# zeux/calm

Hardware: NVIDIA B200
Metric: tok/s single-batch decode (higher is better)
Workload: dtype f32 (fp8 e5m2 weights, f32 accumulate, fp16 KV)

## Files before the change

### calm_b200/csrc/attn.cuh

```cuda
#pragma once

#include "stages.cuh"

#define ATTN2_BP 16
#define ATTN2_MAXB 32

__device__ __forceinline__ void cluster_sync_all() {
	asm volatile("barrier.cluster.arrive.release.aligned;" ::: "memory");
	asm volatile("barrier.cluster.wait.acquire.aligned;" ::: "memory");
}
__device__ __forceinline__ float ld_dsmem(const float* local_ptr, uint32_t cta_rank) {
	uint32_t raddr;
	float v;
	asm volatile("mapa.shared::cluster.u32 %0, %1, %2;" : "=r"(raddr) : "r"(smem_u32(local_ptr)), "r"(cta_rank));
	asm volatile("ld.shared::cluster.f32 %0, [%1];" : "=f"(v) : "r"(raddr) : "memory");
	return v;
}

#define ATTN2_MAX_CLUSTER 16

template <typename KVT>
__host__ __device__ inline size_t attn2_smem_bytes(int hg, int head_dim, int nbmax, int nsplit) {
	size_t kv = (size_t)2 * nbmax * ATTN2_BP * head_dim * sizeof(KVT);
	size_t scratch = (size_t)(ATTN_THREADS / 32) * hg * (head_dim + 2);
	size_t scratch2 = (size_t)(2 * nsplit + 1) * hg;
	if (scratch2 > scratch) scratch = scratch2;
	return kv + ((size_t)hg * head_dim + scratch + (size_t)hg * (head_dim + 2)) * sizeof(float);
}

__device__ __forceinline__ float attn_cell_wait(const unsigned long long* cell, unsigned epoch, int* err) {
	unsigned long long v;
	unsigned spins = 0;
	unsigned long long t0 = 0;
	for (;;) {
		asm volatile("ld.volatile.global.u64 %0, [%1];" : "=l"(v) : "l"(cell) : "memory");
		if ((unsigned)(v >> 32) == epoch) break;
		if ((++spins & 1023) == 0) {
			const unsigned long long now = globaltimer_ns();
			if (!t0) t0 = now;
			if (now - t0 > 5000000000ull) {
				if (err) *reinterpret_cast<volatile int*>(err) = 9200;
				__threadfence_system();
				__trap();
			}
		}
	}
	return __uint_as_float((unsigned)v);
}

__device__ __forceinline__ void attn_cell_pair_wait(const unsigned long long* cell, unsigned epoch, int* err, float& v0, float& v1) {
	unsigned long long c0, c1;
	unsigned spins = 0;
	unsigned long long t0 = 0;
	for (;;) {
		asm volatile("ld.volatile.global.v2.u64 {%0, %1}, [%2];" : "=l"(c0), "=l"(c1) : "l"(cell) : "memory");
		if ((unsigned)(c0 >> 32) == epoch && (unsigned)(c1 >> 32) == epoch) break;
		if ((++spins & 1023) == 0) {
			const unsigned long long now = globaltimer_ns();
			if (!t0) t0 = now;
			if (now - t0 > 5000000000ull) {
				if (err) *reinterpret_cast<volatile int*>(err) = 9201;
				__threadfence_system();
				__trap();
			}
		}
	}
	v0 = __uint_as_float((unsigned)c0), v1 = __uint_as_float((unsigned)c1);
}

template <typename KVT, int HG, int LPP, bool CLUSTER>
__global__ void __launch_bounds__(ATTN_THREADS) k_attn2(const AttnArgs a) {
	typedef typename KvRaw<KVT>::type raw_t;
	constexpr int HD = LPP * 8, P = LPP / HG, G = 32 / LPP, NW = ATTN_THREADS / 32, NC = LPP;
	static_assert(HG * P == LPP && P >= 1 && P <= 4 && ATTN2_BP % P == 0, "unsupported head grouping");
	extern __shared__ __align__(128) unsigned char smem_raw[];
	__shared__ __align__(8) uint64_t bars[ATTN2_MAXB];
	__shared__ int flag;
	const int tid = threadIdx.x, lane = tid & 31, warp = tid >> 5;
	const int nbmax = a.nbmax, nsplit = a.nsplit;
	const int unit = blockIdx.x / nsplit, split = blockIdx.x % nsplit;
	const int kvh = unit / a.qgroups;
	const int hbase = kvh * a.kv_mul + (unit % a.qgroups) * HG;
	constexpr uint32_t BLK = ATTN2_BP * HD * sizeof(KVT);
	KVT* Ks = reinterpret_cast<KVT*>(smem_raw);
	KVT* Vs = Ks + (size_t)nbmax * ATTN2_BP * HD;
	float* qs = reinterpret_cast<float*>(Vs + (size_t)nbmax * ATTN2_BP * HD);
	float* scratch = qs + HG * HD;
	float* myrec = scratch + max(NW * HG * (HD + 2), (2 * nsplit + 1) * HG);
	const KVT* kglob = reinterpret_cast<const KVT*>(a.kc) + (size_t)kvh * a.seq_len * HD;
	const KVT* vglob = reinterpret_cast<const KVT*>(a.vc) + (size_t)kvh * a.seq_len * HD;

#define ATTN_DBG(i)                                                          \
	do {                                                                     \
		if (a.dbg && blockIdx.x == 0 && tid == 0) a.dbg[i] = globaltimer_ns(); \
	} while (0)
	ATTN_DBG(0);
	pdl_launch_next();
	if (tid == 0) {
		for (int j = 0; j < nbmax; ++j) mbar_init(&bars[j], 1);
		mbar_init_fence();
	}
	__syncthreads();
	bool issued = false;
	auto request = [&](int j) {
		const int b = split + j * nsplit;
		const uint32_t bytes = (uint32_t)min(ATTN2_BP, a.seq_len - b * ATTN2_BP) * HD * sizeof(KVT);
		mbar_expect_tx(&bars[j], 2 * bytes);
		tma_load_1d(Ks + (size_t)j * ATTN2_BP * HD, kglob + (size_t)b * ATTN2_BP * HD, bytes, &bars[j]);
		tma_load_1d(Vs + (size_t)j * ATTN2_BP * HD, vglob + (size_t)b * ATTN2_BP * HD, bytes, &bars[j]);
	};
	if (tid < nbmax) {
		const int hint = min(*reinterpret_cast<const volatile int*>(&a.tp->kv_len), a.seq_len);
		if ((split + tid * nsplit) * ATTN2_BP < hint) request(tid), issued = true;
	}
	pdl_wait_prev();
	stamp_begin(a.stamp);
	ATTN_DBG(1);
	if (a.dbg && tid == 0) atomicMin(a.dbg + 10, globaltimer_ns());
	constexpr int QPT = (HG * HD + ATTN_THREADS - 1) / ATTN_THREADS;
	float qreg[QPT];
#pragma unroll
	for (int i = 0; i < QPT; ++i) qreg[i] = (tid + i * ATTN_THREADS < HG * HD) ? __ldcg(a.q + (size_t)hbase * HD + tid + i * ATTN_THREADS) : 0.f;
	const int kv_len = a.tp->kv_len, kv_pos = a.tp->kv_pos, kv_sink = a.tp->kv_sink;
	const unsigned epoch = (unsigned)a.tp->tp_seq * a.epoch_stride + a.epoch_idx;
	if (tid < nbmax && !issued && (split + tid * nsplit) * ATTN2_BP < kv_len) request(tid), issued = true;
#pragma unroll
	for (int i = 0; i < QPT; ++i)
		if (tid + i * ATTN_THREADS < HG * HD) qs[tid + i * ATTN_THREADS] = qreg[i];
	__syncthreads();
	ATTN_DBG(2);

	const int nblk = (kv_len + ATTN2_BP - 1) / ATTN2_BP;
	const int nb = nblk > split ? (nblk - split + nsplit - 1) / nsplit : 0;
	const int nslots = nb * ATTN2_BP;
	const int grp = lane / LPP, li = lane % LPP;

	float acc[HG][8], m[HG], l[HG];
#pragma unroll
	for (int h = 0; h < HG; ++h) {
		m[h] = -FLT_MAX, l[h] = 0.f;
#pragma unroll
		for (int d = 0; d < 8; ++d) acc[h][d] = 0.f;
	}
	float mh = -FLT_MAX, lh = 0.f;

	constexpr int SC = 4, STEP = NW * G * P;
	const int gbase = grp * LPP;
	auto slot_of = [&](int s0, int& j, int& o, int& t0) {
// ... 106 lines not shown
				for (int e = 0; e < 8; ++e) {
					float v = acc[h][e];
#pragma unroll
					for (int i = 0; i < P; ++i) v = fmaf(pw[i], vf[i][e], v);
					acc[h][e] = v;
				}
			}
		}
	}
	ATTN_DBG(4);
#pragma unroll
	for (int h = 0; h < HG; ++h) {
		m[h] = __shfl_sync(0xffffffffu, mh, grp * LPP + h * P);
		l[h] = __shfl_sync(0xffffffffu, lh, grp * LPP + h * P);
	}
	if constexpr (CLUSTER) {
		constexpr int REC = HD + 2;
		__shared__ float mls[ATTN2_MAX_CLUSTER][HG][2];
		__shared__ float invl[HG];
		attn_cta_merge<HG>(a, HG, 0, HG, warp, NW, m, l, acc, scratch, myrec);
		cluster_sync_all();
		for (int i = tid; i < nsplit * HG; i += ATTN_THREADS) {
			const int s = i / HG, h = i % HG;
			mls[s][h][0] = ld_dsmem(myrec + h * REC + HD, s), mls[s][h][1] = ld_dsmem(myrec + h * REC + HD + 1, s);
		}
		__syncthreads();
		if (tid < HG) {
			float M = -FLT_MAX;
			for (int s = 0; s < nsplit; ++s) M = fmaxf(M, mls[s][tid][0]);
			float L = 0.f;
			for (int s = 0; s < nsplit; ++s) {
				const float c = expf(mls[s][tid][0] - M);
				L = fmaf(mls[s][tid][1], c, L);
				mls[s][tid][0] = c;
			}
			invl[tid] = 1.0f / L;
		}
		__syncthreads();
		const int nout = HG * HD, per = (nout + nsplit - 1) / nsplit;
		const int o_end = min(nout, (split + 1) * per);
		for (int o0 = split * per; o0 < o_end; o0 += ATTN_THREADS / 8) {
			const int o = o0 + tid / 8, sg = tid & 7;
			float v = 0.f;
			if (o < o_end) {
				const int h = o / HD, e = o % HD;
				for (int s = sg; s < nsplit; s += 8) v = fmaf(ld_dsmem(myrec + h * REC + e, s), mls[s][h][0], v);
			}
			v += __shfl_xor_sync(0xffffffffu, v, 1), v += __shfl_xor_sync(0xffffffffu, v, 2), v += __shfl_xor_sync(0xffffffffu, v, 4);
			if (o < o_end && sg == 0) __stcg(a.out + (size_t)hbase * HD + o, v * invl[o / HD]);
		}
		cluster_sync_all();
	} else {
		constexpr int REC = HD + 2;
		__shared__ float mls[ATTN2_MAXB + 4][HG][2];
		__shared__ float invl[HG];
		(void)flag;
		attn_cta_merge<HG>(a, HG, 0, HG, warp, NW, m, l, acc, scratch, myrec);
		__syncthreads();
		ATTN_DBG(5);
		unsigned long long* cells = a.cells + (size_t)unit * nsplit * HG * REC;
		for (int i = tid; i < HG * REC; i += ATTN_THREADS) {
			const unsigned long long c = ((unsigned long long)epoch << 32) | __float_as_uint(myrec[i]);
			asm volatile("st.volatile.global.u64 [%0], %1;" ::"l"(cells + (size_t)split * HG * REC + i), "l"(c) : "memory");
		}
		for (int i = tid; i < nsplit * HG; i += ATTN_THREADS) {
			const int s = i / HG, h = i % HG;
			const unsigned long long* c = cells + (size_t)s * HG * REC + h * REC + HD;
			if (s == split) mls[s][h][0] = myrec[h * REC + HD], mls[s][h][1] = myrec[h * REC + HD + 1];
			else attn_cell_pair_wait(c, epoch, a.err, mls[s][h][0], mls[s][h][1]);
		}
		__syncthreads();
		__shared__ float cfs[ATTN2_MAXB + 4][HG];
		for (int i = tid; i < nsplit * HG; i += ATTN_THREADS) {
			const int s = i / HG, h = i % HG;
			float M = -FLT_MAX;
			for (int s2 = 0; s2 < nsplit; ++s2) M = fmaxf(M, mls[s2][h][0]);
			cfs[s][h] = expf(mls[s][h][0] - M);
		}
		__syncthreads();
		if (tid < HG) {
			float L = 0.f;
			for (int s = 0; s < nsplit; ++s) L = fmaf(mls[s][tid][1], cfs[s][tid], L);
			invl[tid] = 1.0f / L;
		}
		for (int i = tid; i < nsplit * HG; i += ATTN_THREADS) mls[i / HG][i % HG][0] = cfs[i / HG][i % HG];
		__syncthreads();
		ATTN_DBG(6);
		const int nout = HG * HD, per = (nout + nsplit - 1) / nsplit;
		const int o_end = min(nout, (split + 1) * per);
		for (int o0 = split * per; o0 < o_end; o0 += ATTN_THREADS / 8) {
			const int o = o0 + tid / 8, sg = tid & 7;
			float v = 0.f;
			if (o < o_end) {
				const int h = o / HD, e = o % HD;
				constexpr int NS8 = (ATTN2_MAXB + 4 + 7) / 8;
				unsigned long long c[NS8];
#pragma unroll
				for (int k = 0; k < NS8; ++k) {
					const int s = sg + 8 * k;
					c[k] = 0;
					if (s < nsplit && s != split) asm volatile("ld.volatile.global.u64 %0, [%1];" : "=l"(c[k]) : "l"(cells + (size_t)s * HG * REC + h * REC + e) : "memory");
				}
#pragma unroll
				for (int k = 0; k < NS8; ++k) {
					const int s = sg + 8 * k;
					if (s < nsplit) {
						float x;
						if (s == split) x = myrec[h * REC + e];
						else if ((unsigned)(c[k] >> 32) == epoch) x = __uint_as_float((unsigned)c[k]);
						else x = attn_cell_wait(cells + (size_t)s * HG * REC + h * REC + e, epoch, a.err);
						v = fmaf(x, mls[s][h][0], v);
					}
				}
			}
			v += __shfl_xor_sync(0xffffffffu, v, 1), v += __shfl_xor_sync(0xffffffffu, v, 2), v += __shfl_xor_sync(0xffffffffu, v, 4);
			if (o < o_end && sg == 0) __stcg(a.out + (size_t)hbase * HD + o, v * invl[o / HD]);
		}
	}
	if (tid < nbmax && issued) mbar_wait(&bars[tid], 0);
	ATTN_DBG(7);
	if (a.dbg && tid == 0) atomicMax(a.dbg + 9, globaltimer_ns());
	stamp_end(a.stamp);
}
```

### calm_b200/csrc/engine.cu

```cuda

#include "../../include/calm_b200.h"

#include <dlfcn.h>
#include <math.h>
#include <string.h>

#include <vector>

#include "stages.cuh"
#include "attn.cuh"
#include "ring.cuh"
#include "prefill.cuh"

namespace {

#define MAX_STAMPS (2 + 5 * MAX_LAYERS)
#define TP_MAX_CAND 2048
enum Stage { ST_EMBED, ST_QKV, ST_ATTN, ST_WO, ST_FFN_UP, ST_FFN_DOWN, ST_OUTPUT, ST_COUNT };
const char* const kStageNames[ST_COUNT] = {"embed", "matmul_qkv", "attention", "matmul_attn", "matmul_ffn_up", "matmul_ffn_down", "output"};

struct Engine {
	bool ready = false;
	int device = -1;
	int sms = 0;
	cudaStream_t stream = nullptr;
	struct Config cfg;
	struct Weights w;
	int kvbits = 16;
	int nact = 1;
	int q_dim = 0, kv_dim = 0, kv_mul = 1;

	float *x = nullptr, *xb = nullptr, *q = nullptr, *att = nullptr, *hb = nullptr, *logits_dev = nullptr;
	float* logits_host = nullptr;
	void *kc = nullptr, *vc = nullptr;
	float* rope_freq = nullptr;
	float2* rope_cs = nullptr;
	unsigned long long* attn_cells = nullptr;
	int* dev_err = nullptr;
	float* attn_partial = nullptr;
	unsigned* attn_counter = nullptr;
	MoeSel* moe_sel = nullptr;
	TokenParams* tp = nullptr;
	float* cand_val = nullptr;
	int* cand_idx = nullptr;
	int* out_tokens = nullptr;
	int out_tokens_cap = 0;
	int* last_token = nullptr;
	int ncand = 0;

	int attn_hg = 1, attn_qgroups = 1, attn_nsplit = 1, attn_lpp = 1;
	int ring_up_ns = 2, ring_up_cps = 2, ring_res_ns = 2, ring_res_warps = 16;
	int ring_up_u = 0, ring_wo_u = 0, ring_down_u = 0, ring_wo_s = 1, ring_down_s = 1;
	int grid_up_ring = 0, grid_wo_ring = 0, grid_down_ring = 0;
	size_t smem_up_ring = 0, smem_wo_ring = 0, smem_down_ring = 0;
	bool attn2_cluster = false;
	bool attn2 = false;
	int attn_nbmax = 0;
	size_t attn2_smem = 0;

	int grid_qkv = 0, grid_wo = 0, grid_up = 0, grid_down = 0, grid_out = 0;
	size_t smem_dim = 0, smem_qdim = 0, smem_hidden = 0;
	int cur_kv_len = 0;
	int cur_pos = 0;
	int attn_nsplit_cap = 1 << 30;

	bool pf_kv = false;
	bool pf_attn_wo = false;
	size_t pf_attn_up = 0;
	size_t pf_wo_up = 0;
	size_t pf_up_down = 0;
	bool pf_down_qkv = false;


	int tp_rank = 0, tp_world = 1;
	void* tp_comm = nullptr;
	float* xpart = nullptr;
	bool tp_fused = false;
	size_t up_expert_stride = 0;
	int out_row0 = 0, out_row1 = 0;
	size_t tp_off_logits = 0, tp_off_cval = 0, tp_off_cidx = 0, tp_off_flags = 0;
	void* tp_area = nullptr;
	void* tp_peer[TP_MAX_WORLD] = {};
	int* tp_err = nullptr;
	std::vector<void*> tp_owned;


	cudaGraphExec_t graph[2][5] = {};
	int graph_launches[2][5] = {};
	SampleState* sample_state = nullptr;
	int sample_chunks = 0;
	int* sample_count = nullptr;
	float* sample_csum = nullptr;
	int* sample_idx = nullptr;
	float* sample_prob = nullptr;
	bool use_graph = true;
	bool use_pdl = true;
	int carveout = -1;

	bool perf = false;
	bool debug = false;
	unsigned long long* stamps = nullptr;
	unsigned long long* stamp_acc = nullptr;
	int n_stamps = 0;
	int stamp_stage[MAX_STAMPS] = {};
	double stamp_bytes[MAX_STAMPS] = {};
	double stage_ms[ST_COUNT] = {};
	double stage_bytes[ST_COUNT] = {};
	long stage_launches[ST_COUNT] = {};
	double token_span_ms = 0;
	int perf_runs = 0;
	cudaEvent_t timer[2] = {nullptr, nullptr};
// ... 235 lines not shown
void launch_attn(const AttnArgs& a, int nunits, int* nl) {
	const size_t smem = attn_smem(HG, a.head_dim, a.nsplit);
	if (!nl) {
		smem_optin(k_attn<KVT, HG>, smem);
		return;
	}
	launch_pdl(k_attn<KVT, HG>, nunits * a.nsplit, ATTN_THREADS, smem, a);
	++*nl;
}

template <typename KVT, int HG, int LPP>
void launch_attn2(const AttnArgs& a, int nunits, int* nl) {
	if (!nl) {
		smem_optin(k_attn2<KVT, HG, LPP, false>, g.attn2_smem);
		{
			int per_sm = 0;
			CUDA_CHECK(cudaOccupancyMaxActiveBlocksPerMultiprocessor(&per_sm, k_attn2<KVT, HG, LPP, false>, ATTN_THREADS, g.attn2_smem));
			if (per_sm * g.sms < nunits * a.nsplit) g.attn2 = false;
		}
		if (g.attn2_cluster) {
			smem_optin(k_attn2<KVT, HG, LPP, true>, g.attn2_smem);
			if (a.nsplit > 8) CUDA_CHECK(cudaFuncSetAttribute(k_attn2<KVT, HG, LPP, true>, cudaFuncAttributeNonPortableClusterSizeAllowed, 1));
			cudaLaunchConfig_t cfg = {};
			cfg.gridDim = dim3(nunits * a.nsplit), cfg.blockDim = dim3(ATTN_THREADS), cfg.dynamicSmemBytes = g.attn2_smem;
			cudaLaunchAttribute at[1];
			at[0].id = cudaLaunchAttributeClusterDimension;
			at[0].val.clusterDim.x = a.nsplit, at[0].val.clusterDim.y = 1, at[0].val.clusterDim.z = 1;
			cfg.attrs = at, cfg.numAttrs = 1;
			int nclusters = 0;
			if (cudaOccupancyMaxActiveClusters(&nclusters, k_attn2<KVT, HG, LPP, true>, &cfg) != cudaSuccess || nclusters < 1) {
				(void)cudaGetLastError();
				g.attn2_cluster = false;
			}
		}
		return;
	}
	if (g.attn2_cluster) {
		same_carveout((const void*)k_attn2<KVT, HG, LPP, true>);
		cudaLaunchConfig_t cfg = {};
		cfg.gridDim = dim3(nunits * a.nsplit), cfg.blockDim = dim3(ATTN_THREADS), cfg.dynamicSmemBytes = g.attn2_smem, cfg.stream = g.stream;
		cudaLaunchAttribute at[2];
		at[0].id = cudaLaunchAttributeProgrammaticStreamSerialization;
		at[0].val.programmaticStreamSerializationAllowed = g.use_pdl ? 1 : 0;
		at[1].id = cudaLaunchAttributeClusterDimension;
		at[1].val.clusterDim.x = a.nsplit, at[1].val.clusterDim.y = 1, at[1].val.clusterDim.z = 1;
		cfg.attrs = at, cfg.numAttrs = 2;
		CUDA_CHECK(cudaLaunchKernelEx(&cfg, k_attn2<KVT, HG, LPP, true>, a));
	} else {
		launch_pdl(k_attn2<KVT, HG, LPP, false>, nunits * a.nsplit, ATTN_THREADS, g.attn2_smem, a);
	}
	++*nl;
}

bool attn2_shape_ok(int hg, int lpp, int head_dim) {
	return head_dim == lpp * 8 && ((lpp == 16 && (hg == 4 || hg == 8)) || (lpp == 8 && (hg == 2 || hg == 4 || hg == 8)));
}

template <typename KVT>
void dispatch_attn(const AttnArgs& a, int nunits, int* nl) {
	if (g.attn2) {
		switch (g.attn_lpp * 100 + g.attn_hg) {
		case 1604: launch_attn2<KVT, 4, 16>(a, nunits, nl); return;
		case 1608: launch_attn2<KVT, 8, 16>(a, nunits, nl); return;
		case 802: launch_attn2<KVT, 2, 8>(a, nunits, nl); return;
		case 804: launch_attn2<KVT, 4, 8>(a, nunits, nl); return;
		case 808: launch_attn2<KVT, 8, 8>(a, nunits, nl); return;
		}
	}
	switch (g.attn_hg) {
	case 1: launch_attn<KVT, 1>(a, nunits, nl); break;
	case 2: launch_attn<KVT, 2>(a, nunits, nl); break;
	case 3: launch_attn<KVT, 3>(a, nunits, nl); break;
	case 4: launch_attn<KVT, 4>(a, nunits, nl); break;
	case 5: launch_attn<KVT, 5>(a, nunits, nl); break;
	case 6: launch_attn<KVT, 6>(a, nunits, nl); break;
	case 7: launch_attn<KVT, 7>(a, nunits, nl); break;
	default: launch_attn<KVT, 8>(a, nunits, nl); break;
	}
}

template <int DBITS, int U, int NS>
void ring_up_launch(const FfnUpArgs& a, bool attr_only) {
	if (attr_only) return smem_optin(k_ffn_up_ring<DBITS, U, NS>, g.smem_up_ring);
	launch_pdl(k_ffn_up_ring<DBITS, U, NS>, g.grid_up_ring, 256, g.smem_up_ring, a);
}
template <int DBITS, int U, int NS>
void ring_res_launch(const MatResArgs& a, int S, int grid, size_t smem, bool attr_only) {
	if (attr_only) return smem_optin(k_matres_ring<DBITS, U, NS>, smem);
	launch_pdl(k_matres_ring<DBITS, U, NS>, grid, g.ring_res_warps * 32, smem, a, S);
}
template <int DBITS>
void ring_up_dispatch(const FfnUpArgs& a, bool attr_only) {
	switch (g.ring_up_u * 10 + g.ring_up_ns) {
	case 22: return ring_up_launch<DBITS, 2, 2>(a, attr_only);
	case 23: return ring_up_launch<DBITS, 2, 3>(a, attr_only);
	case 24: return ring_up_launch<DBITS, 2, 4>(a, attr_only);
	case 42: return ring_up_launch<DBITS, 4, 2>(a, attr_only);
	case 43: return ring_up_launch<DBITS, 4, 3>(a, attr_only);
	default: return ring_up_launch<DBITS, 4, 4>(a, attr_only);
	}
}
template <int DBITS>
void ring_res_dispatch(const MatResArgs& a, int u, int S, int grid, size_t smem, bool attr_only) {
	switch (u * 10 + g.ring_res_ns) {
	case 22: return ring_res_launch<DBITS, 2, 2>(a, S, grid, smem, attr_only);
	case 23: return ring_res_launch<DBITS, 2, 3>(a, S, grid, smem, attr_only);
	case 24: return ring_res_launch<DBITS, 2, 4>(a, S, grid, smem, attr_only);
	case 42: return ring_res_launch<DBITS, 4, 2>(a, S, grid, smem, attr_only);
	case 43: return ring_res_launch<DBITS, 4, 3>(a, S, grid, smem, attr_only);
	default: return ring_res_launch<DBITS, 4, 4>(a, S, grid, smem, attr_only);
	}
}
// ... 179 lines not shown
void tp_shard_model() {
	Config& c = g.cfg;
	Weights& w = g.w;
	const int N = g.tp_world, r = g.tp_rank;
	const int ne = c.n_experts ? c.n_experts : 1;
	if (c.n_heads % N || c.n_kv_heads % N || c.hidden_dim % (32 * N)) CALM_FATAL("tensor parallelism: %d ranks do not divide heads %d/%d or hidden %d", N, c.n_heads, c.n_kv_heads, c.hidden_dim);
	const size_t wb = (size_t)w.dbits;
	const int q_dim = c.head_dim * c.n_heads, kv_dim = c.head_dim * c.n_kv_heads;
	const int ql = q_dim / N, kl = kv_dim / N, hl = c.hidden_dim / N;
	auto rows = [&](void* base, size_t row0, size_t cols) { return (void*)((char*)base + row0 * cols * wb / 8); };
	auto col_slice = [&](const void* base, int nrows, size_t cols, size_t col0, size_t ncols) {
		void* dst = dev_alloc((size_t)nrows * ncols * wb / 8);
		CUDA_CHECK(cudaMemcpy2D(dst, ncols * wb / 8, (const char*)base + col0 * wb / 8, cols * wb / 8, ncols * wb / 8, nrows, cudaMemcpyDeviceToDevice));
		g.tp_owned.push_back(dst);
		return dst;
	};
	for (int l = 0; l < c.n_layers; ++l) {
		w.wq[l] = rows(w.wq[l], (size_t)r * ql, c.dim);
		w.wk[l] = rows(w.wk[l], (size_t)r * kl, c.dim);
		w.wv[l] = rows(w.wv[l], (size_t)r * kl, c.dim);
		w.w1[l] = rows(w.w1[l], (size_t)r * hl, c.dim);
		w.w3[l] = rows(w.w3[l], (size_t)r * hl, c.dim);
		w.wo[l] = col_slice(w.wo[l], c.dim, q_dim, (size_t)r * ql, ql);
		w.w2[l] = col_slice(w.w2[l], ne * c.dim, c.hidden_dim, (size_t)r * hl, hl);
		if (w.bqkv[l]) {
			float* b = (float*)dev_alloc((size_t)(ql + 2 * kl) * sizeof(float));
			CUDA_CHECK(cudaMemcpy(b, w.bqkv[l] + (size_t)r * ql, ql * sizeof(float), cudaMemcpyDeviceToDevice));
			CUDA_CHECK(cudaMemcpy(b + ql, w.bqkv[l] + q_dim + (size_t)r * kl, kl * sizeof(float), cudaMemcpyDeviceToDevice));
			CUDA_CHECK(cudaMemcpy(b + ql + kl, w.bqkv[l] + q_dim + kv_dim + (size_t)r * kl, kl * sizeof(float), cudaMemcpyDeviceToDevice));
			g.tp_owned.push_back(b);
			w.bqkv[l] = b;
		}
	}
	if (c.n_experts) g.up_expert_stride = (size_t)c.hidden_dim * c.dim * wb / 8 / 16;
	c.n_heads /= N, c.n_kv_heads /= N, c.hidden_dim = hl;
}

template <int DBITS, typename KVT>
void make_plan() {
	const Config& c = g.cfg;
	g.smem_dim = xs_bytes<DBITS>(c.dim);
	g.smem_qdim = xs_bytes<DBITS>(g.q_dim);
	g.smem_hidden = xs_bytes<DBITS>(c.hidden_dim);
	size_t smem_res = g.smem_qdim > g.smem_hidden ? g.smem_qdim : g.smem_hidden;
	if (smem_res > 227 * 1024 || g.smem_dim > 227 * 1024) CALM_FATAL("activation vector does not fit in shared memory (dim %d, hidden %d)", c.dim, c.hidden_dim);
	smem_optin(k_qkv<DBITS, KVT>, g.smem_dim), smem_optin(k_ffn_up<DBITS>, g.smem_dim), smem_optin(k_output<DBITS>, g.smem_dim);
	smem_optin(k_matres<DBITS>, smem_res);
	{
		g.attn_nbmax = cdiv(cdiv(c.seq_len, ATTN2_BP), g.attn_nsplit);
		g.attn2_smem = attn2_smem_bytes<KVT>(g.attn_hg, c.head_dim, g.attn_nbmax, g.attn_nsplit);
		const bool want = !(getenv("CALM_B200_ATTN2") && atoi(getenv("CALM_B200_ATTN2")) == 0);
		g.attn2 = want && attn2_shape_ok(g.attn_hg, g.attn_lpp, c.head_dim) && g.attn_nbmax <= ATTN2_MAXB && g.attn2_smem <= 200 * 1024;
		g.attn2_cluster = g.attn2 && g.attn_nsplit <= ATTN2_MAX_CLUSTER && getenv("CALM_B200_ATTN_CLUSTER") && atoi(getenv("CALM_B200_ATTN_CLUSTER")) != 0;
		AttnArgs aa = {};
		aa.head_dim = c.head_dim, aa.nsplit = g.attn_nsplit;
		dispatch_attn<KVT>(aa, c.n_kv_heads * g.attn_qgroups, nullptr);
	}
	g.grid_qkv = balanced_grid(cdiv((g.q_dim + 2 * g.kv_dim) / 2, 8), max_ctas(k_qkv<DBITS, KVT>, QKV_THREADS, g.smem_dim));
	g.grid_wo = balanced_grid(cdiv(c.dim / 2, 8), max_ctas(k_matres<DBITS>, 256, g.smem_qdim));
	g.grid_down = balanced_grid(cdiv(c.dim / 2, 8), max_ctas(k_matres<DBITS>, 256, g.smem_hidden));
	if (g.tp_fused) {
		for (int grid : {g.grid_wo, g.grid_down})
			if (cdiv(c.dim / 2, grid * 8) > TP_MAX_ITERS) CALM_FATAL("tensor parallelism: grid %d outside the exchange tables for dim %d", grid, c.dim);
	}
	g.grid_up = imin(max_ctas(k_ffn_up<DBITS>, 256, g.smem_dim), cdiv(g.nact * c.hidden_dim, 8));
	g.ring_up_u = g.ring_wo_u = g.ring_down_u = 0;
	{
		const int hint = getenv("CALM_B200_RING_HINT") ? atoi(getenv("CALM_B200_RING_HINT")) : 1;
		CUDA_CHECK(cudaMemcpyToSymbol(d_ring_l2_hint, &hint, sizeof(int)));
	}
	if (const char* e = getenv("CALM_B200_RING")) sscanf(e, "%d,%d,%d,%d", &g.ring_up_ns, &g.ring_up_cps, &g.ring_res_ns, &g.ring_res_warps);
	const bool ring_ok = c.n_experts == 0;
	const bool ring_up_on = ring_ok && g.ring_up_ns >= 2 && g.ring_up_ns <= RING_MAX_NS;
	const bool ring_res_on = ring_ok && (g.tp_world == 1 || g.tp_fused)  && g.ring_res_ns >= 2 && g.ring_res_ns <= RING_MAX_NS && (g.ring_res_warps == 8 || g.ring_res_warps == 16);
	auto chunk_units = [](size_t rowbytes) { return rowbytes % 2048 == 0 ? 4 : (rowbytes % 1024 == 0 ? 2 : 0); };
	if (ring_up_on) {
		const int u = chunk_units((size_t)c.dim * DBITS / 8);
		if (u) {
			g.smem_up_ring = ring_smem_bytes<DBITS>(c.dim, u, g.ring_up_ns, 8);
			if (g.smem_up_ring <= 200 * 1024) {
				g.ring_up_u = u;
				g.grid_up_ring = imin(g.sms * imin(g.ring_up_cps, (int)(220 * 1024 / g.smem_up_ring)), c.hidden_dim);
				if (g.grid_up_ring < 1) g.grid_up_ring = 1;
				FfnUpArgs fa = {};
				ring_up_dispatch<DBITS>(fa, true);
			}
		}
	}
	if (ring_res_on) {
		auto plan_res = [&](int n, int& u_out, int& s_out, int& grid_out, size_t& smem_out) {
			const size_t rowbytes = (size_t)n * DBITS / 8;
			int u = chunk_units(rowbytes);
			if (u == 4 && getenv("CALM_B200_RING_RES_U") && atoi(getenv("CALM_B200_RING_RES_U")) == 2) u = 2;
			if (!u) return;
			size_t smem = ring_smem_bytes<DBITS>(n, u, g.ring_res_ns, g.ring_res_warps);
			if (smem > 220 * 1024 && u == 4) u = 2, smem = ring_smem_bytes<DBITS>(n, u, g.ring_res_ns, g.ring_res_warps);
			if (smem > 220 * 1024) return;
			const int grid = imin(g.sms * imin(16 / g.ring_res_warps, (int)(224 * 1024 / smem)), c.dim / 2);
			const int cpt = (int)(rowbytes / (u * 512));
			if (g.tp_world > 1 && cdiv(c.dim / 2, grid) + 1 > RING_MAX_PAIRS) return;
			const bool split = cdiv(c.dim / 2, grid) + 1 <= RING_MAX_PAIRS && cpt <= RING_MAX_SLICES;
			u_out = u, s_out = split ? 1 : cpt, grid_out = grid < 1 ? 1 : grid, smem_out = smem;
			MatResArgs ma = {};
			ring_res_dispatch<DBITS>(ma, u, s_out, grid_out, smem, true);
		};
		int uw = 0, ud = 0, sw = 1, sd = 1, gw = 0, gd = 0;
// ... 769 lines not shown
```

Measured before the change: 458.6.

## Add tensor-core mma.sync attention kernel for 4-head groups with 128-dim heads

Adds a new split-KV decode attention kernel that computes QK^T and PV with m16n8k16 fp16 mma.sync and ldmatrix instead of scalar FMA loops. Query and softmax probabilities are split into hi/lo fp16 pairs to keep near-f32 accuracy, and KV rows are TMA-loaded into padded smem rows to avoid bank conflicts. The cross-split cell merge is factored into a shared helper reused by both kernels. The new kernel is enabled by default when the head group is 4, head_dim is 128, the non-cluster attn2 path is active, and occupancy covers all CTAs. It adds extra mma work for the split terms, and fp8 operands go through byte-permute conversion.

```diff
diff --git a/calm_b200/csrc/attn.cuh b/calm_b200/csrc/attn.cuh
--- a/calm_b200/csrc/attn.cuh
+++ b/calm_b200/csrc/attn.cuh
@@ -66,6 +66,73 @@
 		}
 	}
 	v0 = __uint_as_float((unsigned)c0), v1 = __uint_as_float((unsigned)c1);
+}
+
+#define ATTN_DBG(i)                                                                    \
+	do {                                                                               \
+		if (a.dbg && blockIdx.x == 0 && threadIdx.x == 0) a.dbg[i] = globaltimer_ns(); \
+	} while (0)
+
+template <int HG, int HD>
+__device__ __forceinline__ void attn_cell_fold(const AttnArgs& a, int unit, int split, int hbase, unsigned epoch, const float* myrec) {
+	constexpr int REC = HD + 2;
+	__shared__ float mls[ATTN2_MAXB + 4][HG][2];
+	__shared__ float invl[HG];
+	const int tid = threadIdx.x, nsplit = a.nsplit;
+	const unsigned long long* cells = a.cells + (size_t)unit * nsplit * HG * REC;
+	for (int i = tid; i < nsplit * HG; i += ATTN_THREADS) {
+		const int s = i / HG, h = i % HG;
+		const unsigned long long* c = cells + (size_t)s * HG * REC + h * REC + HD;
+		if (s == split) mls[s][h][0] = myrec[h * REC + HD], mls[s][h][1] = myrec[h * REC + HD + 1];
+		else attn_cell_pair_wait(c, epoch, a.err, mls[s][h][0], mls[s][h][1]);
+	}
+	__syncthreads();
+	__shared__ float cfs[ATTN2_MAXB + 4][HG];
+	for (int i = tid; i < nsplit * HG; i += ATTN_THREADS) {
+		const int s = i / HG, h = i % HG;
+		float M = -FLT_MAX;
+		for (int s2 = 0; s2 < nsplit; ++s2) M = fmaxf(M, mls[s2][h][0]);
+		cfs[s][h] = expf(mls[s][h][0] - M);
+	}
+	__syncthreads();
+	if (tid < HG) {
+		float L = 0.f;
+		for (int s = 0; s < nsplit; ++s) L = fmaf(mls[s][tid][1], cfs[s][tid], L);
+		invl[tid] = 1.0f / L;
+	}
+	for (int i = tid; i < nsplit * HG; i += ATTN_THREADS) mls[i / HG][i % HG][0] = cfs[i / HG][i % HG];
+	__syncthreads();
+	ATTN_DBG(6);
+	const int nout = HG * HD, per = (nout + nsplit - 1) / nsplit;
+	const int o_end = min(nout, (split + 1) * per);
+	for (int o0 = split * per; o0 < o_end; o0 += ATTN_THREADS / 8) {
+		const int o = o0 + tid / 8, sg = tid & 7;
+		float v = 0.f;
+		if (o < o_end) {
+			const int h = o / HD, e = o % HD;
+			constexpr int NS8 = (ATTN2_MAXB + 4 + 7) / 8;
+			unsigned long long c[NS8];
+#pragma unroll
+			for (int k = 0; k < NS8; ++k) {
+				const int s = sg + 8 * k;
+				c[k] = 0;
+				if (s < nsplit && s != split) asm volatile("ld.volatile.global.u64 %0, [%1];" : "=l"(c[k]) : "l"(cells + (size_t)s * HG * REC + h * REC + e) : "memory");
+			}
+#pragma unroll
+			for (int k = 0; k < NS8; ++k) {
+				const int s = sg + 8 * k;
+				if (s < nsplit) {
+					float x;
+					if (s == split) x = myrec[h * REC + e];
+					else if ((unsigned)(c[k] >> 32) == epoch) x = __uint_as_float((unsigned)c[k]);
+					else x = attn_cell_wait(cells + (size_t)s * HG * REC + h * REC + e, epoch, a.err);
+					v = fmaf(x, mls[s][h][0], v);
+				}
+			}
+		}
+		v += __shfl_xor_sync(0xffffffffu, v, 1), v += __shfl_xor_sync(0xffffffffu, v, 2), v += __shfl_xor_sync(0xffffffffu, v, 4);
+		if (o < o_end && sg == 0) __stcg(a.out + (size_t)hbase * HD + o, v * invl[o / HD]);
+	}
 }
 
 template <typename KVT, int HG, int LPP, bool CLUSTER>
@@ -90,10 +157,6 @@
 	const KVT* kglob = reinterpret_cast<const KVT*>(a.kc) + (size_t)kvh * a.seq_len * HD;
 	const KVT* vglob = reinterpret_cast<const KVT*>(a.vc) + (size_t)kvh * a.seq_len * HD;
 
-#define ATTN_DBG(i)                                                          \
-	do {                                                                     \
-		if (a.dbg && blockIdx.x == 0 && tid == 0) a.dbg[i] = globaltimer_ns(); \
-	} while (0)
 	ATTN_DBG(0);
 	pdl_launch_next();
 	if (tid == 0) {
@@ -306,8 +369,6 @@
 		cluster_sync_all();
 	} else {
 		constexpr int REC = HD + 2;
-		__shared__ float mls[ATTN2_MAXB + 4][HG][2];
-		__shared__ float invl[HG];
 		(void)flag;
 		attn_cta_merge<HG>(a, HG, 0, HG, warp, NW, m, l, acc, scratch, myrec);
 		__syncthreads();
@@ -317,62 +378,264 @@
 			const unsigned long long c = ((unsigned long long)epoch << 32) | __float_as_uint(myrec[i]);
 			asm volatile("st.volatile.global.u64 [%0], %1;" ::"l"(cells + (size_t)split * HG * REC + i), "l"(c) : "memory");
 		}
-		for (int i = tid; i < nsplit * HG; i += ATTN_THREADS) {
-			const int s = i / HG, h = i % HG;
-			const unsigned long long* c = cells + (size_t)s * HG * REC + h * REC + HD;
-			if (s == split) mls[s][h][0] = myrec[h * REC + HD], mls[s][h][1] = myrec[h * REC + HD + 1];
-			else attn_cell_pair_wait(c, epoch, a.err, mls[s][h][0], mls[s][h][1]);
-		}
-		__syncthreads();
-		__shared__ float cfs[ATTN2_MAXB + 4][HG];
-		for (int i = tid; i < nsplit * HG; i += ATTN_THREADS) {
-			const int s = i / HG, h = i % HG;
-			float M = -FLT_MAX;
-			for (int s2 = 0; s2 < nsplit; ++s2) M = fmaxf(M, mls[s2][h][0]);
-			cfs[s][h] = expf(mls[s][h][0] - M);
-		}
-		__syncthreads();
-		if (tid < HG) {
-			float L = 0.f;
-			for (int s = 0; s < nsplit; ++s) L = fmaf(mls[s][tid][1], cfs[s][tid], L);
-			invl[tid] = 1.0f / L;
-		}
-		for (int i = tid; i < nsplit * HG; i += ATTN_THREADS) mls[i / HG][i % HG][0] = cfs[i / HG][i % HG];
-		__syncthreads();
-		ATTN_DBG(6);
-		const int nout = HG * HD, per = (nout + nsplit - 1) / nsplit;
-		const int o_end = min(nout, (split + 1) * per);
-		for (int o0 = split * per; o0 < o_end; o0 += ATTN_THREADS / 8) {
-			const int o = o0 + tid / 8, sg = tid & 7;
-			float v = 0.f;
-			if (o < o_end) {
-				const int h = o / HD, e = o % HD;
-				constexpr int NS8 = (ATTN2_MAXB + 4 + 7) / 8;
-				unsigned long long c[NS8];
-#pragma unroll
-				for (int k = 0; k < NS8; ++k) {
-					const int s = sg + 8 * k;
-					c[k] = 0;
-					if (s < nsplit && s != split) asm volatile("ld.volatile.global.u64 %0, [%1];" : "=l"(c[k]) : "l"(cells + (size_t)s * HG * REC + h * REC + e) : "memory");
-				}
-#pragma unroll
-				for (int k = 0; k < NS8; ++k) {
-					const int s = sg + 8 * k;
-					if (s < nsplit) {
-						float x;
-						if (s == split) x = myrec[h * REC + e];
-						else if ((unsigned)(c[k] >> 32) == epoch) x = __uint_as_float((unsigned)c[k]);
-						else x = attn_cell_wait(cells + (size_t)s * HG * REC + h * REC + e, epoch, a.err);
-						v = fmaf(x, mls[s][h][0], v);
-					}
-				}
-			}
-			v += __shfl_xor_sync(0xffffffffu, v, 1), v += __shfl_xor_sync(0xffffffffu, v, 2), v += __shfl_xor_sync(0xffffffffu, v, 4);
-			if (o < o_end && sg == 0) __stcg(a.out + (size_t)hbase * HD + o, v * invl[o / HD]);
-		}
+		attn_cell_fold<HG, HD>(a, unit, split, hbase, epoch, myrec);
 	}
 	if (tid < nbmax && issued) mbar_wait(&bars[tid], 0);
 	ATTN_DBG(7);
 	if (a.dbg && tid == 0) atomicMax(a.dbg + 9, globaltimer_ns());
 	stamp_end(a.stamp);
 }
+
+#define ATTN_MMA_HG 4
+#define ATTN_MMA_HD 128
+
+template <typename KVT>
+struct AttnMmaShape {
+	static constexpr int ROWB = ATTN_MMA_HD * (int)sizeof(KVT);
+	static constexpr int KST = ROWB + 16;
+};
+
+__host__ __device__ inline int attn_mma_sst(int nbmax) { return (nbmax * ATTN2_BP + 31) / 32 * 32 + 8; }
+__host__ __device__ inline int attn_mma_pst(int nbmax) { return (nbmax * ATTN2_BP / 2 + 31) / 32 * 32 + 4; }
+template <typename KVT>
+__host__ __device__ inline size_t attn_mma_smem_bytes(int nbmax) {
+	return (size_t)2 * nbmax * ATTN2_BP * AttnMmaShape<KVT>::KST +
+	       ((size_t)ATTN_MMA_HG * attn_mma_sst(nbmax) + (size_t)2 * ATTN_MMA_HG * attn_mma_pst(nbmax) + (size_t)ATTN_MMA_HG * (ATTN_MMA_HD + 2)) * sizeof(float);
+}
+
+__device__ __forceinline__ void mma_f16_16816(float (&c)[4], const uint32_t (&a)[4], uint32_t b0, uint32_t b1) {
+	asm volatile("mma.sync.aligned.m16n8k16.row.col.f32.f16.f16.f32 {%0, %1, %2, %3}, {%4, %5, %6, %7}, {%8, %9}, {%0, %1, %2, %3};"
+	             : "+f"(c[0]), "+f"(c[1]), "+f"(c[2]), "+f"(c[3])
+	             : "r"(a[0]), "r"(a[1]), "r"(a[2]), "r"(a[3]), "r"(b0), "r"(b1));
+}
+__device__ __forceinline__ void ldsm_x4(uint32_t (&r)[4], const void* p) {
+	asm volatile("ldmatrix.sync.aligned.m8n8.x4.shared.b16 {%0, %1, %2, %3}, [%4];" : "=r"(r[0]), "=r"(r[1]), "=r"(r[2]), "=r"(r[3]) : "r"(smem_u32(p)));
+}
+__device__ __forceinline__ void ldsm_x4_trans(uint32_t (&r)[4], const void* p) {
+	asm volatile("ldmatrix.sync.aligned.m8n8.x4.trans.shared.b16 {%0, %1, %2, %3}, [%4];" : "=r"(r[0]), "=r"(r[1]), "=r"(r[2]), "=r"(r[3]) : "r"(smem_u32(p)));
+}
+__device__ __forceinline__ uint32_t pack_half2(__half lo, __half hi) {
+	return (uint32_t)__half_as_ushort(lo) | ((uint32_t)__half_as_ushort(hi) << 16);
+}
+
+template <typename KVT>
+__global__ void __launch_bounds__(ATTN_THREADS, 1) k_attn_mma(const AttnArgs a) {
+	constexpr int HG = ATTN_MMA_HG, HD = ATTN_MMA_HD, BP = ATTN2_BP, NW = ATTN_THREADS / 32, REC = HD + 2;
+	constexpr bool F16 = sizeof(KVT) == 2;
+	constexpr int ROWB = AttnMmaShape<KVT>::ROWB, KST = AttnMmaShape<KVT>::KST;
+	static_assert(NW * 16 == HD, "one warp per 16 output dims");
+	extern __shared__ __align__(128) unsigned char smem_raw[];
+	__shared__ __align__(8) uint64_t bars[ATTN2_MAXB];
+	__shared__ int s_hint;
+	__shared__ float s_m[HG], s_l[NW];
+	__shared__ __align__(16) float s_q[HG * HD];
+	const int tid = threadIdx.x, lane = tid & 31, warp = tid >> 5, g = lane >> 2, t = lane & 3;
+	const int nbmax = a.nbmax, nsplit = a.nsplit, seq_len = a.seq_len;
+	const int unit = blockIdx.x / nsplit, split = blockIdx.x % nsplit;
+	const int kvh = unit / a.qgroups;
+	const int hbase = kvh * a.kv_mul + (unit % a.qgroups) * HG;
+	const int sst = attn_mma_sst(nbmax), pst = attn_mma_pst(nbmax);
+	unsigned char* Ks = smem_raw;
+	unsigned char* Vs = Ks + (size_t)nbmax * BP * KST;
+	float* sc = reinterpret_cast<float*>(Vs + (size_t)nbmax * BP * KST);
+	uint32_t* ph = reinterpret_cast<uint32_t*>(sc + HG * sst);
+	float* myrec = reinterpret_cast<float*>(ph + 2 * HG * pst);
+	const unsigned char* kglob = reinterpret_cast<const unsigned char*>(a.kc) + (size_t)kvh * seq_len * ROWB;
+	const unsigned char* vglob = reinterpret_cast<const unsigned char*>(a.vc) + (size_t)kvh * seq_len * ROWB;
+
+	ATTN_DBG(0);
+	pdl_launch_next();
+	if (tid == 0) {
+		for (int j = 0; j < nbmax; ++j) mbar_init(&bars[j], 1);
+		mbar_init_fence();
+		s_hint = min(*reinterpret_cast<const volatile int*>(&a.tp->kv_len), seq_len);
+	}
+	__syncthreads();
+	auto request_row = [&](int j, int r) {
+		const int b = split + j * nsplit;
+		const int rows = min(BP, seq_len - b * BP);
+		if (r == 0) mbar_expect_tx(&bars[j], (uint32_t)(2 * rows * ROWB));
+		if (r < rows) {
+			const size_t src = ((size_t)b * BP + r) * ROWB, dst = ((size_t)j * BP + r) * KST;
+			tma_load_1d(Ks + dst, kglob + src, ROWB, &bars[j]);
+			tma_load_1d(Vs + dst, vglob + src, ROWB, &bars[j]);
+		}
+	};
+	const int hint = s_hint;
+	auto early = [&](int j) { return (split + j * nsplit) * BP < hint; };
+	for (int i = tid; i < nbmax * BP; i += ATTN_THREADS)
+		if (early(i / BP)) request_row(i / BP, i % BP);
+	pdl_wait_prev();
+	stamp_begin(a.stamp);
+	ATTN_DBG(1);
+	if (a.dbg && tid == 0) atomicMin(a.dbg + 10, globaltimer_ns());
+
+	static_assert(HG * HD == 2 * ATTN_THREADS, "one float2 of q per thread");
+	const float2 qg = __ldcg(reinterpret_cast<const float2*>(a.q + (size_t)hbase * HD) + tid);
+	const int kv_len = a.tp->kv_len, kv_pos = a.tp->kv_pos, kv_sink = a.tp->kv_sink;
+	const unsigned epoch = (unsigned)a.tp->tp_seq * a.epoch_stride + a.epoch_idx;
+	auto needed = [&](int j) { return (split + j * nsplit) * BP < kv_len; };
+	for (int i = tid; i < nbmax * BP; i += ATTN_THREADS)
+		if (!early(i / BP) && needed(i / BP)) request_row(i / BP, i % BP);
+	reinterpret_cast<float2*>(s_q)[tid] = qg;
+	__syncthreads();
+	const int qh = g >> 1;
+	float2 qv[8][2];
+#pragma unroll
+	for (int kk = 0; kk < 8; ++kk) {
+		const int d0 = F16 ? 16 * kk + 2 * t : 16 * kk + 4 * t, d1 = F16 ? d0 + 8 : d0 + 2;
+		qv[kk][0] = *reinterpret_cast<const float2*>(s_q + qh * HD + d0);
+		qv[kk][1] = *reinterpret_cast<const float2*>(s_q + qh * HD + d1);
+	}
+	uint32_t qb[8][2];
+	int qexp;
+	{
+		float mx = 0.f;
+#pragma unroll
+		for (int kk = 0; kk < 8; ++kk)
+			mx = fmaxf(mx, fmaxf(fmaxf(fabsf(qv[kk][0].x), fabsf(qv[kk][0].y)), fmaxf(fabsf(qv[kk][1].x), fabsf(qv[kk][1].y))));
+		mx = fmaxf(mx, __shfl_xor_sync(0xffffffffu, mx, 1)), mx = fmaxf(mx, __shfl_xor_sync(0xffffffffu, mx, 2));
+		frexpf(mx, &qexp);
+		qexp = max(-100, min(qexp, 100));
+		const float s = ldexpf(1.f, 15 - qexp);
+		auto split_q = [&](float x) {
+			const float y = x * s;
+			const __half hi = __float2half_rn(y);
+			return (g & 1) ? __float2half_rn(y - __half2float(hi)) : hi;
+		};
+#pragma unroll
+		for (int kk = 0; kk < 8; ++kk)
+#pragma unroll
+			for (int i = 0; i < 2; ++i) qb[kk][i] = pack_half2(split_q(qv[kk][i].x), split_q(qv[kk][i].y));
+	}
+	const float sunscale = ldexpf(1.f, __shfl_sync(0xffffffffu, qexp, 8 * t) - 15);
+	ATTN_DBG(2);
+
+	const int nblk = (kv_len + BP - 1) / BP;
+	const int nb = nblk > split ? (nblk - split + nsplit - 1) / nsplit : 0;
+	const int nslots = nb * BP;
+
+	for (int j = warp; j < nb; j += NW) {
+		mbar_wait(&bars[j], 0);
+		if (j == 0) ATTN_DBG(3);
+		const int p0 = (split + j * nsplit) * BP;
+		unsigned char* kb = Ks + (size_t)j * BP * KST;
+		unsigned char* vb = Vs + (size_t)j * BP * KST;
+		if ((kv_pos >= p0 && kv_pos < p0 + BP) || p0 < kv_sink || p0 + BP > kv_len) {
+			for (int o = 0; o < BP; ++o) {
+				const int pos = p0 + o;
+				const bool fresh = pos < kv_len && (pos == kv_pos || pos < kv_sink), past = pos >= kv_len;
+				if ((fresh || past) && lane < ROWB / 16) {
+					uint4 kr = make_uint4(0, 0, 0, 0), vr = kr;
+					if (fresh) {
+						kr = __ldcg(reinterpret_cast<const uint4*>(kglob + (size_t)pos * ROWB) + lane);
+						vr = __ldcg(reinterpret_cast<const uint4*>(vglob + (size_t)pos * ROWB) + lane);
+					}
+					reinterpret_cast<uint4*>(kb + o * KST)[lane] = kr;
+					reinterpret_cast<uint4*>(vb + o * KST)[lane] = vr;
+				}
+			}
+			__syncwarp();
+		}
+		float c[4] = {0.f, 0.f, 0.f, 0.f};
+		if constexpr (F16) {
+			const unsigned char* base = kb + ((lane & 7) + ((lane >> 3) & 1) * 8) * KST + (lane >> 4) * 16;
+#pragma unroll
+			for (int kk = 0; kk < 8; ++kk) {
+				uint32_t af[4];
+				ldsm_x4(af, base + kk * 32);
+				mma_f16_16816(c, af, qb[kk][0], qb[kk][1]);
+			}
+		} else {
+			const unsigned char* base = kb + ((lane & 7) + ((lane >> 3) & 1) * 8) * KST + (lane >> 4) * 16;
+#pragma unroll
+			for (int s2 = 0; s2 < 4; ++s2) {
+				uint32_t r[4];
+				ldsm_x4(r, base + s2 * 32);
+#pragma unroll
+				for (int h = 0; h < 2; ++h) {
+					const uint32_t af[4] = {__byte_perm(0u, r[2 * h], 0x5040), __byte_perm(0u, r[2 * h + 1], 0x5040), __byte_perm(0u, r[2 * h], 0x7060),
+					                        __byte_perm(0u, r[2 * h + 1], 0x7060)};
+					mma_f16_16816(c, af, qb[2 * s2 + h][0], qb[2 * s2 + h][1]);
+				}
+			}
+		}
+#pragma unroll
+		for (int i = 0; i < 2; ++i) {
+			const int o = g + 8 * i;
+			sc[t * sst + j * BP + o] = p0 + o < kv_len ? (c[2 * i] + c[2 * i + 1]) * sunscale * a.inv_sqrt_hd : -FLT_MAX;
+		}
+	}
+	__syncthreads();
+
+	{
+		const int h = warp & 3, half = warp >> 2;
+		const float* sh = sc + h * sst;
+		float m = -FLT_MAX;
+		for (int i = lane; i < nslots; i += 32) m = fmaxf(m, sh[i]);
+#pragma unroll
+		for (int o = 16; o >= 1; o >>= 1) m = fmaxf(m, __shfl_xor_sync(0xffffffffu, m, o));
+		float ls = 0.f;
+		for (int i = half * 32 + lane; i < nslots / 2; i += 64) {
+			const float2 s2 = *reinterpret_cast<const float2*>(sh + 2 * i);
+			const float e0 = __expf(s2.x - m), e1 = __expf(s2.y - m);
+			ls += e0 + e1;
+			const __half h0 = __float2half_rn(e0), h1 = __float2half_rn(e1);
+			ph[(2 * h) * pst + i] = pack_half2(h0, h1);
+			ph[(2 * h + 1) * pst + i] = pack_half2(__float2half_rn(e0 - __half2float(h0)), __float2half_rn(e1 - __half2float(h1)));
+		}
+#pragma unroll
+		for (int o = 16; o >= 1; o >>= 1) ls += __shfl_xor_sync(0xffffffffu, ls, o);
+		if (lane == 0) {
+			s_l[warp] = ls;
+			if (half == 0) s_m[h] = m;
+		}
+	}
+	__syncthreads();
+
+	float acc0[4] = {0.f, 0.f, 0.f, 0.f}, acc1[4] = {0.f, 0.f, 0.f, 0.f};
+	auto pv = [&](int j, float (&acc)[4]) {
+		const unsigned char* vb = Vs + (size_t)j * BP * KST;
+		uint32_t af[4];
+		if constexpr (F16) {
+			ldsm_x4_trans(af, vb + ((lane & 7) + (lane >> 4) * 8) * KST + (16 * warp + ((lane >> 3) & 1) * 8) * 2);
+		} else {
+			const unsigned char* col = vb + 16 * warp + 2 * g;
+			uint32_t x[4];
+#pragma unroll
+			for (int i = 0; i < 4; ++i) x[i] = *reinterpret_cast<const unsigned short*>(col + (2 * t + (i & 1) + 8 * (i >> 1)) * KST);
+			af[0] = __byte_perm(x[0], x[1], 0x4202), af[1] = __byte_perm(x[0], x[1], 0x5212);
+			af[2] = __byte_perm(x[2], x[3], 0x4202), af[3] = __byte_perm(x[2], x[3], 0x5212);
+		}
+		const uint32_t* pb = ph + g * pst + j * (BP / 2) + t;
+		mma_f16_16816(acc, af, pb[0], pb[4]);
+	};
+	for (int j = 0; j < nb; j += 2) {
+		pv(j, acc0);
+		if (j + 1 < nb) pv(j + 1, acc1);
+	}
+	ATTN_DBG(4);
+
+	{
+		const int r0 = F16 ? 16 * warp + g : 16 * warp + 2 * g, r1 = F16 ? r0 + 8 : r0 + 1;
+		const float v0 = (acc0[0] + acc0[1]) + (acc1[0] + acc1[1]), v1 = (acc0[2] + acc0[3]) + (acc1[2] + acc1[3]);
+		unsigned long long* cell = a.cells + ((size_t)unit * nsplit + split) * HG * REC + t * REC;
+		asm volatile("st.volatile.global.u64 [%0], %1;" ::"l"(cell + r0), "l"(((unsigned long long)epoch << 32) | __float_as_uint(v0)) : "memory");
+		asm volatile("st.volatile.global.u64 [%0], %1;" ::"l"(cell + r1), "l"(((unsigned long long)epoch << 32) | __float_as_uint(v1)) : "memory");
+		myrec[t * REC + r0] = v0, myrec[t * REC + r1] = v1;
+		if (tid < HG) {
+			const float m = s_m[tid], l = s_l[tid] + s_l[tid + 4];
+			unsigned long long* ml = a.cells + ((size_t)unit * nsplit + split) * HG * REC + tid * REC + HD;
+			asm volatile("st.volatile.global.u64 [%0], %1;" ::"l"(ml), "l"(((unsigned long long)epoch << 32) | __float_as_uint(m)) : "memory");
+			asm volatile("st.volatile.global.u64 [%0], %1;" ::"l"(ml + 1), "l"(((unsigned long long)epoch << 32) | __float_as_uint(l)) : "memory");
+			myrec[tid * REC + HD] = m, myrec[tid * REC + HD + 1] = l;
+		}
+	}
+	__syncthreads();
+	ATTN_DBG(5);
+	attn_cell_fold<HG, HD>(a, unit, split, hbase, epoch, myrec);
+	if (tid < nbmax && (early(tid) || needed(tid))) mbar_wait(&bars[tid], 0);
+	ATTN_DBG(7);
+	if (a.dbg && tid == 0) atomicMax(a.dbg + 9, globaltimer_ns());
+	stamp_end(a.stamp);
+}
diff --git a/calm_b200/csrc/engine.cu b/calm_b200/csrc/engine.cu
--- a/calm_b200/csrc/engine.cu
+++ b/calm_b200/csrc/engine.cu
@@ -55,8 +55,9 @@
 	size_t smem_up_ring = 0, smem_wo_ring = 0, smem_down_ring = 0;
 	bool attn2_cluster = false;
 	bool attn2 = false;
+	bool attn_mma = false;
 	int attn_nbmax = 0;
-	size_t attn2_smem = 0;
+	size_t attn2_smem = 0, attn_mma_smem = 0;
 
 	int grid_qkv = 0, grid_wo = 0, grid_up = 0, grid_down = 0, grid_out = 0;
 	size_t smem_dim = 0, smem_qdim = 0, smem_hidden = 0;
@@ -398,12 +399,29 @@
 	++*nl;
 }
 
+template <typename KVT>
+void launch_attn_mma(const AttnArgs& a, int nunits, int* nl) {
+	if (!nl) {
+		smem_optin(k_attn_mma<KVT>, g.attn_mma_smem);
+		int per_sm = 0;
+		CUDA_CHECK(cudaOccupancyMaxActiveBlocksPerMultiprocessor(&per_sm, k_attn_mma<KVT>, ATTN_THREADS, g.attn_mma_smem));
+		if (per_sm * g.sms < nunits * a.nsplit) g.attn_mma = false;
+		return;
+	}
+	launch_pdl(k_attn_mma<KVT>, nunits * a.nsplit, ATTN_THREADS, g.attn_mma_smem, a);
+	++*nl;
+}
+
 bool attn2_shape_ok(int hg, int lpp, int head_dim) {
 	return head_dim == lpp * 8 && ((lpp == 16 && (hg == 4 || hg == 8)) || (lpp == 8 && (hg == 2 || hg == 4 || hg == 8)));
 }
 
 template <typename KVT>
 void dispatch_attn(const AttnArgs& a, int nunits, int* nl) {
+	if (g.attn_mma) {
+		launch_attn_mma<KVT>(a, nunits, nl);
+		if (nl) return;
+	}
 	if (g.attn2) {
 		switch (g.attn_lpp * 100 + g.attn_hg) {
 		case 1604: launch_attn2<KVT, 4, 16>(a, nunits, nl); return;
@@ -689,6 +707,9 @@
 		const bool want = !(getenv("CALM_B200_ATTN2") && atoi(getenv("CALM_B200_ATTN2")) == 0);
 		g.attn2 = want && attn2_shape_ok(g.attn_hg, g.attn_lpp, c.head_dim) && g.attn_nbmax <= ATTN2_MAXB && g.attn2_smem <= 200 * 1024;
 		g.attn2_cluster = g.attn2 && g.attn_nsplit <= ATTN2_MAX_CLUSTER && getenv("CALM_B200_ATTN_CLUSTER") && atoi(getenv("CALM_B200_ATTN_CLUSTER")) != 0;
+		g.attn_mma_smem = attn_mma_smem_bytes<KVT>(g.attn_nbmax);
+		const bool want_mma = !(getenv("CALM_B200_ATTN_MMA") && atoi(getenv("CALM_B200_ATTN_MMA")) == 0);
+		g.attn_mma = want_mma && g.attn2 && !g.attn2_cluster && g.attn_hg == ATTN_MMA_HG && c.head_dim == ATTN_MMA_HD && g.attn_mma_smem <= 200 * 1024;
 		AttnArgs aa = {};
 		aa.head_dim = c.head_dim, aa.nsplit = g.attn_nsplit;
 		dispatch_attn<KVT>(aa, c.n_kv_heads * g.attn_qgroups, nullptr);
```

Measured after the change: 488.0, median of 6. 6.4% higher.
